# shenwei356/bio

Measured on AMD Instinct MI355X. Metric: Gbases/s hashed (k=21 ntHash + minimizer), higher is better.
Workload: dtype u64

## Files before the change

bio_amd/csrc/kernels_pk.hpp:

```cpp
#pragma once
#include <utility>

#include "kernels_fast.hpp"

namespace bsk {

template <int... Is, class F>
__device__ __forceinline__ void pk_unroll_impl(std::integer_sequence<int, Is...>, F &&f) {
    (f(std::integral_constant<int, Is>{}), ...);
}
template <int N, class F>
__device__ __forceinline__ void pk_unroll(F &&f) {
    pk_unroll_impl(std::make_integer_sequence<int, N>{}, f);
}

#ifndef BSK_PK_ROWS
#define BSK_PK_ROWS 58
#endif
struct PkLds {
    static constexpr int PR = BSK_PK_ROWS;
    static constexpr int ROW = 33;
    static constexpr int TAB = 0;
    static constexpr int TAB2 = 320;
    static constexpr int NHEADS = (32 * (PR - 1)) / 64 + 2;
    static constexpr int HEADS = 0;
    static constexpr int CTAB = 256;
    static constexpr int SH = 768;
    static constexpr int SP = SH + (PR + 1) * ROW * 8;
    static constexpr int TOTAL = (SP + (PR + 1) * ROW * 2 + 15) & ~15;
    static_assert(NHEADS * 8 <= CTAB && CTAB + 512 <= SH && TAB2 + 256 <= SH && TOTAL <= 20480, "PkLds");
};

struct PkTabs {
    u32x4 row;
    u32 at;
    __device__ __forceinline__ void init(int k, int lane, u32 tab = (u32)PkLds::TAB, u32 tab2 = (u32)PkLds::TAB2) {
        row = (u32x4){0, 0, 0, 0};
        at = 0xffffffffu;
        if (lane < 20) {
            const unsigned out = (unsigned)lane >> 2, in = (unsigned)lane & 3u;
            u64 f = seed_fwd_code(in);
            u64 r = rol64(seed_rev_code(in), (unsigned)(k - 1));
            if (out < 4) {
                f ^= rol64(seed_fwd_code(out), (unsigned)k);
                r ^= ror64(seed_rev_code(out), 1);
            }
            row = (u32x4){(u32)f, (u32)(f >> 32), (u32)r, (u32)(r >> 32)};
            at = tab + (u32)lane * 16u;
        } else if (lane >= 32 && lane < 48) {
            const unsigned c0 = (unsigned)lane & 3u, c1 = ((unsigned)lane >> 2) & 3u;
            const u64 f = rol64(seed_fwd_code(c0), 1) ^ seed_fwd_code(c1);
            const u64 r = ror64(rol64(seed_rev_code(c0), (unsigned)(k - 1)), 1) ^ rol64(seed_rev_code(c1), (unsigned)(k - 1));
            row = (u32x4){(u32)f, (u32)(f >> 32), (u32)r, (u32)(r >> 32)};
            at = tab2 + (u32)(lane - 32) * 16u;
        }
    }
    __device__ __forceinline__ void write(LDSQ char *ldsq) const {
        if (at != 0xffffffffu) *reinterpret_cast<LDSQ u32x4 *>(ldsq + at) = row;
        wave_sync_lds();
    }
};

template <int W>
struct PkCfg {
    static constexpr int XC = W > 12 ? 4 : W;
};

#define PKNW 16
typedef u32 u32x16 __attribute__((ext_vector_type(16)));
struct PkWords {
    u32x4 a, b, c, d;
};
__device__ __forceinline__ PkWords pk_load_words(const u32 *p) {
    PkWords r;
    asm volatile("global_load_dwordx4 %0, %4, off\n\tglobal_load_dwordx4 %1, %4, off offset:16\n\t"
                 "global_load_dwordx4 %2, %4, off offset:32\n\tglobal_load_dwordx4 %3, %4, off offset:48"
                 : "=&v"(r.a), "=&v"(r.b), "=&v"(r.c), "=&v"(r.d)
                 : "v"(p));
    return r;
}
__device__ __forceinline__ u64 pk_load_u64(const u64 *p) {
    u64 r;
    asm volatile("global_load_dwordx2 %0, %1, off" : "=&v"(r) : "v"(p));
    return r;
}
__device__ __forceinline__ void pk_wait_loads(u64 &d0, u64 &d1) { asm volatile("s_waitcnt vmcnt(0)" : "+v"(d0), "+v"(d1)::"memory"); }
__device__ __forceinline__ void pk_wait_loads(PkWords &p) { asm volatile("s_waitcnt vmcnt(0)" : "+v"(p.a), "+v"(p.b), "+v"(p.c), "+v"(p.d)::"memory"); }
__device__ __forceinline__ void pk_ticket_async(u32 *ticket, u32 &t) {
    u64 ex;
    asm volatile("s_mov_b64 %1, exec\n\ts_mov_b64 exec, 1\n\tglobal_atomic_add %0, %2, %3, off sc0\n\ts_mov_b64 exec, %1"
                 : "+v"(t), "=&s"(ex)
                 : "v"(ticket), "v"(1u)
                 : "memory");
}
__device__ __forceinline__ void pk_wait_loads(PkWords &p, u64 &d0, u32 &f, u32 &t) {
    asm volatile("s_waitcnt vmcnt(0)" : "+v"(p.a), "+v"(p.b), "+v"(p.c), "+v"(p.d), "+v"(d0), "+v"(f), "+v"(t)::"memory");
}
__device__ __forceinline__ u32 pk_load_u8(const u8 *p) {
    u32 r;
    asm volatile("global_load_ubyte %0, %1, off" : "=&v"(r) : "v"(p));
    return r;
}
template <int W, bool LONG, class LY_ = PkLds, bool RINGM = false, bool SELM = false>
struct PkMin {
    typedef LY_ LY;
    const u32 *__restrict__ w;
    LDSQ char *lds;
    int k, lane;
    u32 nk;
    u32 fl, fh_, rl, rh_;
    u32 S[W];
    u64 H[W];
    u32 SB[W];
    u32 P, bm, tmin;
    u32 nsel;
    u32 slot, spare;
    u32 glo, gspan;
    u32 c8000;
    int sstep;
    u32 send;
    u32 in_lo, in_hi, out_lo, out_hi;
    u32x4 pw;
    u32x16 wr;
    static constexpr bool POS2 = !RINGM && !SELM;
    u32 i2;

    __device__ __forceinline__ void set_words(const PkWords &p) {
        wr = (u32x16){p.a.x, p.a.y, p.a.z, p.a.w, p.b.x, p.b.y, p.b.z, p.b.w, p.c.x, p.c.y, p.c.z, p.c.w, p.d.x, p.d.y, p.d.z, p.d.w};
    }
    __device__ __forceinline__ void word2(u32 i, u32 &lo, u32 &hi) const {
        const u32 iu = (u32)__builtin_amdgcn_readfirstlane((int)i);
        if (!LONG || iu + 1 < (u32)PKNW) {
            lo = wr[iu], hi = wr[iu + 1];
        } else {
            lo = w[iu], hi = w[iu + 1];
        }
    }
    __device__ __forceinline__ u32 word(u32 i) const {
        const u32 iu = (u32)__builtin_amdgcn_readfirstlane((int)i);
        if constexpr (RINGM) {
            if (iu < 4u) return iu == 0 ? pw.x : iu == 1 ? pw.y : iu == 2 ? pw.z : pw.w;
            return w[iu];
        }
        if (!LONG || iu < (u32)PKNW) return wr[iu];
        return w[iu];
    }
    __device__ __forceinline__ void load_block_words(u32 i0) {
        const u32 t0 = i0 + (u32)k - 1, p0 = i0 - 1;
        in_lo = w[t0 >> 4];
        in_hi = w[(t0 >> 4) + 1];
        out_lo = w[p0 >> 4];
        out_hi = w[(p0 >> 4) + 1];
    }
    __device__ __forceinline__ void load_block0_words() {
        const u32 t0 = (u32)k - 1;
        in_lo = word(t0 >> 4);
        in_hi = word((t0 >> 4) + 1);
        out_lo = word(0);
        out_hi = word(1);
    }
    __device__ __forceinline__ void roll(u32x4 x) {
        const u32 a = __builtin_amdgcn_alignbit(fl, fh_, 31), b = __builtin_amdgcn_alignbit(fh_, fl, 31);
        const u32 c = __builtin_amdgcn_alignbit(rh_, rl, 1), d = __builtin_amdgcn_alignbit(rl, rh_, 1);
        fl = a ^ x.x;
        fh_ = b ^ x.y;
        rl = c ^ x.z;
        rh_ = d ^ x.w;
    }
    __device__ __forceinline__ void roll2(u32x4 x) {
        const u32 a = __builtin_amdgcn_alignbit(fl, fh_, 30), b = __builtin_amdgcn_alignbit(fh_, fl, 30);
        const u32 c = __builtin_amdgcn_alignbit(rh_, rl, 2), d = __builtin_amdgcn_alignbit(rl, rh_, 2);
        fl = a ^ x.x;
        fh_ = b ^ x.y;
        rl = c ^ x.z;
        rh_ = d ^ x.w;
    }

    __device__ __forceinline__ void guard() {
        if constexpr (RINGM || SELM) return;
        const bool in = slot - glo <= gspan;
        slot = in ? slot : spare;
        sstep = in ? sstep : 0;
    }
    template <int IDX, int O>
    __device__ __forceinline__ void emit(u32 pbase) {
        if constexpr (!SELM) emit_staged<IDX, O>(pbase);
    }
    template <int IDX, int O>
    __device__ __forceinline__ void emit_staged(u32 pbase) {
        const u32 b = (bm >> IDX) & 1u;
        u32 pv;
        if constexpr (POS2) {
            (void)pbase;
            pv = SB[O];
        } else {
            asm("v_add3_u32 %0, %1, %2, %3" : "=v"(pv) : "v"(SB[O]), "s"(pbase), "n"(O));
        }
#if defined(PK_MASKST)
        {
            const u32 a0 = (u32)(uintptr_t)(lds + LY::SH) + slot, a1 = (u32)(uintptr_t)(lds + LY::SP) + (slot >> 2);
            u64 sv;
            asm volatile("v_cmp_ne_u32_e32 vcc, 0, %1\n\ts_and_saveexec_b64 %0, vcc\n\tds_write_b64 %2, %3\n\tds_write_b16 %4, %5\n\ts_mov_b64 exec, %0"
                         : "=&s"(sv) : "v"(b), "v"(a0), "v"(H[O]), "v"(a1), "v"(pv) : "vcc", "memory");
        }
#elif defined(PK_NOPOS)
        *reinterpret_cast<LDSQ u64 *>(lds + LY::SH + slot) = H[O];
#ifdef PK_STRMASK
        asm volatile("" ::"v"(pv));
#endif
#elif !defined(PK_NOSTAGE)
        *reinterpret_cast<LDSQ u64 *>(lds + LY::SH + slot) = H[O];
        *reinterpret_cast<LDSQ u16 *>(lds + LY::SP + (slot >> 2)) = (u16)pv;
#else
        asm volatile("" ::"v"(H[O]), "v"(pv), "v"(slot));
#endif
        asm("v_mad_i32_i24 %0, %1, %2, %0" : "+v"(slot) : "v"(b), "v"(sstep));
        if constexpr (RINGM) slot = slot == send ? (u32)lane * 8u : slot;
    }

    template <bool FIRST, bool RAG, int PAR>
    __device__ __forceinline__ void block(u32 i0, u32 okbit, bool suffix) {
        constexpr int CB = PAR * 16, PB = (1 - PAR) * 16;
        constexpr int XC = PkCfg<W>::XC;
        const u32 t0 = i0 + (u32)k - 1, p0 = FIRST ? 0u : i0 - 1u;
        u32 in_lo, in_hi, out_lo, out_hi;
        if constexpr (RINGM) {
            in_lo = this->in_lo, in_hi = this->in_hi, out_lo = this->out_lo, out_hi = this->out_hi;
            load_block_words(i0 + (u32)W);
        } else {
            word2(t0 >> 4, in_lo, in_hi);
            word2(p0 >> 4, out_lo, out_hi);
        }
        const u32 cinb = __builtin_amdgcn_alignbit(in_hi, in_lo, (t0 & 15) * 2);
        u32 coutb;
        if (FIRST) coutb = out_lo << 2;
        else coutb = __builtin_amdgcn_alignbit(out_hi, out_lo, (p0 & 15) * 2);
        const u32 E = (cinb & 0x33333333u) | ((coutb & 0x33333333u) << 2);
        const u32 O = ((cinb >> 2) & 0x33333333u) | (coutb & 0xCCCCCCCCu);
        const u32 E4 = E << 4, O4 = O << 4;
        u32x4 xs[W];
        auto fetch = [&](int o0) {
#pragma unroll
            for (int o = o0; o < o0 + XC && o < W; ++o) {
                const int j = o >> 1;
                const u32 src = (j & 1) ? ((o & 1) ? O : E) : ((o & 1) ? O4 : E4);
                u32 a;
                switch (j >> 1) {
                    case 0: asm("v_and_b32_sdwa %0, %1, %2 dst_sel:DWORD dst_unused:UNUSED_PAD src0_sel:BYTE_0 src1_sel:DWORD" : "=v"(a) : "v"(src), "s"(0xF0u)); break;
                    case 1: asm("v_and_b32_sdwa %0, %1, %2 dst_sel:DWORD dst_unused:UNUSED_PAD src0_sel:BYTE_1 src1_sel:DWORD" : "=v"(a) : "v"(src), "s"(0xF0u)); break;
                    case 2: asm("v_and_b32_sdwa %0, %1, %2 dst_sel:DWORD dst_unused:UNUSED_PAD src0_sel:BYTE_2 src1_sel:DWORD" : "=v"(a) : "v"(src), "s"(0xF0u)); break;
                    default: asm("v_and_b32_sdwa %0, %1, %2 dst_sel:DWORD dst_unused:UNUSED_PAD src0_sel:BYTE_3 src1_sel:DWORD" : "=v"(a) : "v"(src), "s"(0xF0u)); break;
                }
                if (FIRST && o == 0) a = 0x100u | (a & 0x30u);
#ifndef PK_NOTAB
                xs[o] = *reinterpret_cast<LDSQ const u32x4 *>(lds + LY::TAB + a);
#else
                xs[o] = (u32x4){a, a ^ E, a + O, a ^ cinb};
#endif
            }
        };
        fetch(0);
        if (XC < W) fetch(XC);
        const u32 pbase = (u32)__builtin_amdgcn_readfirstlane((int)(i0 - (u32)W));
        if constexpr (POS2) {
            i2 = 2u * i0;
            asm volatile("" : "+v"(i2));
        }
        if (!FIRST) guard();
        u32 vb = 0;
        if (RAG && !FIRST) {
            const int left = (int)nk - (int)i0;
            const u32 nv = (u32)(left < 0 ? 0 : left > W ? W : left);
            vb = (1u << nv) - 1u;
        }
        pk_unroll<W>([&](auto oc) {
            constexpr int o = decltype(oc)::value;
            if (XC < W && o && o % XC == 0 && o + XC < W) {
                __builtin_amdgcn_sched_barrier(0);
                fetch(o + XC);
            }
            roll(xs[o]);
            if (!FIRST) this->template emit<PB + o, o>(pbase);
            const lmask rev = lt64(rl, rh_, fl, fh_);
            const u32 hl = sel(rev, rl, fl), hh = sel(rev, rh_, fh_);
            if constexpr (POS2) {
                lmask co;
                asm("v_addc_co_u32_e64 %0, %1, %2, %3, %4" : "=v"(SB[o]), "=s"(co) : "n"(2 * o), "v"(i2), "s"(rev));
            } else {
                asm("v_cndmask_b32_e64 %0, 0, %1, %2" : "=v"(SB[o]) : "v"(c8000), "s"(rev));
            }
            H[o] = ((u64)hh << 32) | hl;
            u32 pk;
            asm("v_and_or_b32 %0, %1, %2, %3" : "=v"(pk) : "v"(hh), "s"(0xffffffe0u), "n"(CB + o));
            if (o == 0) {
                P = pk;
            } else {
#ifndef PK_NOTIE
                const u32 d = pk ^ P;
                tmin = tmin < d ? tmin : d;
#endif
                P = P < pk ? P : pk;
            }
            if (!FIRST || o == W - 1) {
                u32 m = P;
                if constexpr (o != W - 1) {
#ifndef PK_NOTIE
                    const u32 d = P ^ S[o + 1];
                    tmin = tmin < d ? tmin : d;
#endif
                    m = P < S[o + 1] ? P : S[o + 1];
                }
                u32 one = 1u;
                if (FIRST) one = okbit;
                else if (RAG) one = (vb >> o) & 1u;
                bm |= one << (m & 31u);
            }
            S[o] = pk;
        });
        if (suffix) {
#pragma unroll
            for (int q = W - 2; q >= 0; --q) {
#ifndef PK_NOTIE
                const u32 d = S[q] ^ S[q + 1];
                tmin = tmin < d ? tmin : d;
#endif
                S[q] = S[q] < S[q + 1] ? S[q] : S[q + 1];
            }
        }
        if constexpr (SELM) {
            if (!FIRST) {
                const u32 wsel = (bm >> PB) & ((1u << W) - 1u);
                *reinterpret_cast<LDSQ u32 *>(lds + LY::MASK + (i0 / (u32)W - 1u) * 256u + (u32)lane * 4u) = wsel;
                nsel += (u32)__builtin_popcount(wsel);
            }
        }
        if (!FIRST) bm &= PAR ? 0xffff0000u : 0x0000ffffu;
    }

    template <int PAR>
    __device__ __forceinline__ void drain(u32 i0) {
        if constexpr (SELM) {
            const u32 wsel = (bm >> (PAR * 16)) & ((1u << W) - 1u);
            *reinterpret_cast<LDSQ u32 *>(lds + LY::MASK + (i0 / (u32)W) * 256u + (u32)lane * 4u) = wsel;
            nsel += (u32)__builtin_popcount(wsel);
            return;
        }
        const u32 pbase = (u32)__builtin_amdgcn_readfirstlane((int)i0);
        guard();
        pk_unroll<W>([&](auto oc) {
            constexpr int o = decltype(oc)::value;
            this->template emit<PAR * 16 + o, o>(pbase);
        });
    }

    __device__ __forceinline__ void begin(u32 slot0, int step, u32 col8) {
        fl = fh_ = rl = rh_ = 0;
        bm = 0;
        nsel = 0;
        c8000 = 0x8000u;
        asm volatile("" : "+v"(c8000));
        tmin = 0xffffffffu;
        slot = slot0;
        sstep = step;
        if constexpr (RINGM) {
            (void)col8;
            spare = glo = gspan = 0;
            send = (u32)(LY::ROWS * LY::ROW * 8) + (u32)lane * 8u;
        } else {
            spare = (u32)(LY::PR * LY::ROW * 8) + col8;
            send = 0;
            constexpr u32 RB = (u32)(LY::ROW * 8);
            glo = step < 0 ? col8 + (u32)(W - 1) * RB : col8;
            gspan = (u32)(LY::PR - W) * RB + (step < 0 ? 0u : RB);
        }
        if constexpr (RINGM) load_block0_words();
        for (int t0 = 0; t0 < k - 1; t0 += 16) {
            const u32 word = this->word((u32)t0 >> 4);
            const int nb = (k - 1 - t0) < 16 ? (k - 1 - t0) : 16;
            int j = 0;
            for (; j + 8 <= nb; j += 8) {
                const u32 sub = word >> (2 * j);
                const u32x4 x0 = *reinterpret_cast<LDSQ const u32x4 *>(lds + LY::TAB2 + ((sub & 0xf) << 4));
                const u32x4 x1 = *reinterpret_cast<LDSQ const u32x4 *>(lds + LY::TAB2 + (sub & 0xf0));
                const u32x4 x2 = *reinterpret_cast<LDSQ const u32x4 *>(lds + LY::TAB2 + ((sub & 0xf00) >> 4));
                const u32x4 x3 = *reinterpret_cast<LDSQ const u32x4 *>(lds + LY::TAB2 + ((sub & 0xf000) >> 8));
                roll2(x0);
                roll2(x1);
                roll2(x2);
                roll2(x3);
            }
            for (; j + 2 <= nb; j += 2) roll2(*reinterpret_cast<LDSQ const u32x4 *>(lds + LY::TAB2 + (((word >> (2 * j)) & 0xf) << 4)));
            for (; j < nb; ++j) roll(*reinterpret_cast<LDSQ const u32x4 *>(lds + LY::TAB + 256 + (((word >> (2 * j)) & 3) << 4)));
        }
    }

    __device__ __forceinline__ void run(u32 nk_max, bool ok, u32 nk_min, u32 slot0, int step, u32 col8) {
        begin(slot0, step, col8);
        block<true, false, 0>(0, ok ? 1u : 0u, nk_max > (u32)W);
        u32 i0 = W;
        int last_par = 0;
        for (;;) {
            if (i0 >= nk_max) break;
            {
                const bool more = i0 + W < nk_max;
                if (i0 + W <= nk_min) block<false, false, 1>(i0, 1u, more);
                else block<false, true, 1>(i0, 1u, more);
            }
            i0 += W;
            last_par = 1;
            if (i0 >= nk_max) break;
            {
                const bool more = i0 + W < nk_max;
                if (i0 + W <= nk_min) block<false, false, 0>(i0, 1u, more);
                else block<false, true, 0>(i0, 1u, more);
            }
            i0 += W;
            last_par = 0;
        }
        if (last_par) drain<1>(i0 - W);
        else drain<0>(i0 - W);
    }
};

template <int U, class LY = PkLds, bool POS2 = false>
__device__ __forceinline__ void pk_copyout(char *lds, int lane, u32 cnt, u32 excl, u32 T, u64 base, const KArgs &a) {
    constexpr int NH = LY::NHEADS;
    u64 *s_heads = reinterpret_cast<u64 *>(lds + LY::HEADS);
    u64 *s_tab64 = reinterpret_cast<u64 *>(lds + LY::CTAB);
    const u64 nzmask = __builtin_amdgcn_ballot_w64(cnt > 0);
    if (lane < NH) s_heads[lane] = 0;
    wave_sync_lds();
    if (cnt > 0) {
        constexpr int RB = LY::ROW * 8;
        const int col8 = (lane & 31) * 8;
        const int S = lane < 32 ? RB : -RB;
        const int A = lane < 32 ? col8 - (int)excl * RB : col8 + ((int)(LY::PR - 1) + (int)excl) * RB;
        const u32 rk = __builtin_amdgcn_mbcnt_hi((u32)(nzmask >> 32), __builtin_amdgcn_mbcnt_lo((u32)nzmask, 0));
        s_tab64[rk] = ((u64)(u32)S << 32) | (u32)A;
        if (excl) atomicOr(&s_heads[(excl - 1u) >> 6], 1ULL << ((excl - 1u) & 63u));
    }
    wave_sync_lds();
    const u64 hw = lane < NH ? s_heads[lane] : 0ULL;
    const u32 hw_lo = (u32)hw, hw_hi = (u32)(hw >> 32);
    u32 heads_before = 0;
    const char *sh = lds + LY::SH, *sp = lds + LY::SP;
    u64 *const gh = a.hash + base;
    u32 *const gp = a.pos + base;
    auto trip = [&](u32 t0, auto check) {
        constexpr bool CHECK = decltype(check)::value;
        u32 rank[U];
#pragma unroll
        for (int j = 0; j < U; ++j) {
            const u32 c = (t0 >> 6) + j;
            const u32 mlo = (u32)__builtin_amdgcn_readlane((int)hw_lo, (int)c), mhi = (u32)__builtin_amdgcn_readlane((int)hw_hi, (int)c);
            rank[j] = (__builtin_amdgcn_mbcnt_hi(mhi, __builtin_amdgcn_mbcnt_lo(mlo, 0u)) << 3) + (heads_before << 3);
            heads_before += (u32)__builtin_popcountll(((u64)mhi << 32) | mlo);
        }
        u64 ent[U];
#pragma unroll
        for (int j = 0; j < U; ++j) ent[j] = *reinterpret_cast<const u64 *>(reinterpret_cast<const char *>(s_tab64) + rank[j]);
        if constexpr (U == 8) {
            __builtin_amdgcn_sched_barrier(0);
            asm volatile("" ::"v"(ent[0]), "v"(ent[1]), "v"(ent[2]), "v"(ent[3]), "v"(ent[4]), "v"(ent[5]), "v"(ent[6]), "v"(ent[7]));
            __builtin_amdgcn_sched_barrier(0);
        }
        u64 hv[U];
        u32 pv[U];
#pragma unroll
        for (int j = 0; j < U; ++j) {
            const u32 t = t0 + 64 * j + lane;
            const int off = __mul24((int)t, (int)(u32)(ent[j] >> 32)) + (int)(u32)ent[j];
            const u32 so = (!CHECK || t < T) ? (u32)off : 0u;
            hv[j] = *reinterpret_cast<const u64 *>(sh + so);
            if constexpr (POS2) pv[j] = *reinterpret_cast<const u16 *>(sp + (so >> 2));
            else pv[j] = (u32)(int)*reinterpret_cast<const short *>(sp + (so >> 2));
        }
        if constexpr (U == 8) {
            __builtin_amdgcn_sched_barrier(0);
            asm volatile("" ::"v"(hv[0]), "v"(hv[1]), "v"(hv[2]), "v"(hv[3]), "v"(hv[4]), "v"(hv[5]), "v"(hv[6]), "v"(hv[7]), "v"(pv[0]), "v"(pv[1]),
                         "v"(pv[2]), "v"(pv[3]), "v"(pv[4]), "v"(pv[5]), "v"(pv[6]), "v"(pv[7]));
            __builtin_amdgcn_sched_barrier(0);
        }
#pragma unroll
        for (int j = 0; j < U; ++j) {
            const u32 t = t0 + 64 * j + lane;
#ifdef PK_NOSTORE
            asm volatile("" ::"v"(hv[j]), "v"(pv[j]));
#else
            if (!CHECK || t < T) {
#ifndef PK_NOHASHST
                __builtin_nontemporal_store(hv[j], &gh[t]);
#else
                asm volatile("" ::"v"(hv[j]));
#endif
#ifndef PK_NOPOSST
                __builtin_nontemporal_store(POS2 ? __builtin_amdgcn_alignbit(pv[j], pv[j], 1) : pv[j] & 0x80007fffu, &gp[t]);
#else
                asm volatile("" ::"v"(pv[j]));
#endif
            }
#endif
        }
    };
    u32 t0 = 0;
    for (; t0 + 64 * U <= T; t0 += 64 * U) trip(t0, std::false_type{});
    if (t0 < T) trip(t0, std::true_type{});
    wave_sync_lds();
}

#ifndef PK_TICKET
#define PK_TICKET 8u
#endif
template <int W, bool LONG>
__global__ __launch_bounds__(64, 2) void k_minimizer_pk(KArgs a) {
    typedef PkLds LY;
    __shared__ __attribute__((aligned(16))) char lds[LY::TOTAL];
    LDSQ char *const ldsq = (LDSQ char *)lds;
    const int lane = lane_id();
    PkTabs tabs;
    tabs.init(a.k, lane);
#ifdef PK_STAGGER
    for (u32 i = (((blockIdx.x * 2654435761u) >> 24) * (u32)PK_STAGGER) >> 8; i; --i) __builtin_amdgcn_s_sleep(32);
#endif
    const u64 slab = (u64)64 * BSK_FAST_CAP;
    const u32 col8 = (u32)(lane & 31) * 8u;
    constexpr u32 RB = (u32)(LY::ROW * 8);
    const u32 top = (u32)(LY::PR - 1) * RB + col8;
    u64 d_n1 = 0, d_cur = 0;
    PkWords pw_cur = {{0, 0, 0, 0}, {0, 0, 0, 0}, {0, 0, 0, 0}, {0, 0, 0, 0}};
    bool have = false;
    const u32 lseg = a.fixcap / a.list_grid;
    u32 lcur = 0;
    const u32 tku = a.tk ? a.tk : PK_TICKET;
    const bool ahead = tku >= 3u;
    u32 tv = 0;
    u32 nt = ~0u;
    for (u32 unit = next_ticket(a.ticket, lane) * tku, uend = unit + tku; unit < a.nunits; ++unit, ({
             if (unit == uend) {
                 unit = ahead ? nt : next_ticket(a.ticket, lane) * tku;
                 uend = unit + tku;
             }
         })) {
        const u64 r = (u64)unit * 64 + lane;
        const u64 u2 = (!ahead || unit + 2u < uend) ? (u64)unit + 2u : (u64)nt + (unit + 2u - uend);
        const bool nxt = unit + 1 != uend ? unit + 1 < a.nunits : ahead && nt < a.nunits;
        const bool ask = ahead && unit + 3u == uend;
        const u64 rmax = a.n - 1;
        if (!have) {
            d_cur = pk_load_u64(a.desc + (r < rmax ? r : rmax));
            d_n1 = pk_load_u64(a.desc + (r + 64 < rmax ? r + 64 : rmax));
            pk_wait_loads(d_cur, d_n1);
            pw_cur = pk_load_words(a.words + (d_cur >> 24));
            pk_wait_loads(pw_cur);
        }
        PkWords pw_n1 = pk_load_words(a.words + (d_n1 >> 24));
        const u64 r2 = u2 * 64 + lane;
        u64 d_n2 = pk_load_u64(a.desc + (r2 < rmax ? r2 : rmax));
        u32 rfl = pk_load_u8(a.rflags ? a.rflags + (r < rmax ? r : rmax) : reinterpret_cast<const u8 *>(a.desc));
        if (ask) pk_ticket_async(a.ticket, tv);
        const u64 d = d_cur;
        const PkWords pw = pw_cur;
        const u64 off = d >> 24, L = desc_len(a, d);
        const u64 ro = out_index(a, r, d);
        const bool ok = r < a.n && L >= (u64)a.circ_ext && (L - (u64)a.circ_ext) + 1 >= (u64)a.k + (u64)W;
        const u32 nk = ok ? (u32)(L - a.k + 1) : 0u;
        const u32 nk_max = wave_max_u32(nk);
        const u32 nk_min = ~wave_max_u32(~(ok ? nk : 0xffffffffu));
        u32 cnt = 0, tmin_lane = 0xffffffffu;
        if (nk_max) {
            tabs.write(ldsq);
            PkMin<W, LONG> pm;
            pm.w = a.words + off;
            pm.set_words(pw);
            pm.lds = ldsq;
            pm.k = a.k;
            pm.lane = lane;
            pm.nk = nk;
            const u32 spare = (u32)LY::PR * RB + col8;
            pm.run(nk_max, ok, nk_min, !ok ? spare : lane < 32 ? col8 : top, !ok ? 0 : lane < 32 ? (int)RB : -(int)RB, col8);
            if (ok) cnt = (lane < 32 ? pm.slot - col8 : top - pm.slot) / RB;
            tmin_lane = pm.tmin;
        }
        pk_wait_loads(pw_n1, d_n2, rfl, tv);
        if (ask) nt = (u32)__builtin_amdgcn_readfirstlane((int)tv) * tku;
        d_cur = d_n1;
        pw_cur = pw_n1;
        d_n1 = d_n2;
        have = nxt;
        const u32 cnt_pair = cnt + (u32)__builtin_amdgcn_ds_bpermute((lane ^ 32) * 4, (int)cnt);
        u64 bad = __builtin_amdgcn_ballot_w64(cnt_pair >= (u32)LY::PR);
        u64 tied = __builtin_amdgcn_ballot_w64(ok && tmin_lane < 32u);
#if defined(PK_NOSTAGE) || defined(PK_NOTIE) || defined(PK_NOTAB) || defined(PK_NOCOPY) || defined(PK_NOSTORE) || defined(PK_NOFB)
        bad = 0;
        tied = 0;
#endif
        const u64 redo = bad | tied;
        if (redo) {
            list_append(a, a.rlist, lseg, lcur, redo, lane, r);
            if ((redo >> lane) & 1) cnt = 0;
        }
        const u32 incl = wave_incl_scan_u32(cnt, lane);
        const u32 excl = incl - cnt;
        const u32 T = wave_bcast_u32(incl, 63);
        const u64 base = (u64)unit * slab;
#ifndef PK_NOCOPY
#ifndef PK_CU
#define PK_CU 8
#endif
        if (T) pk_copyout<PK_CU, LY, PkMin<W, LONG>::POS2>(lds, lane, cnt, excl, T, base, a);
#endif
        if (r < a.n) {
            if (!((redo >> lane) & 1)) a.refs[ro] = ((base + excl) << 24) | cnt;
            u8 sbyte = ok ? BSK_ST_OK : BSK_ST_SHORT;
            if (ok && a.rflags) sbyte |= (u8)rfl;
            a.status[ro] = sbyte;
        }
    }
    list_close(a.rlist, lseg, lcur, lane);
}

#ifdef BSK_IMPL_PK
#ifndef BSK_PK_WS
#define BSK_PK_WS(X) X(2) X(3) X(4) X(5) X(6) X(7) X(8) X(9) X(10) X(11) X(12) X(13)
#endif
bool pk_minimizer_supported(int w) { return w >= 2 && w <= 13; }
u32 pk_minimizer_short_bases() { return 16u * (PKNW - 1); }
int pk_minimizer_blocks_per_cu(int w) {
    int nb = 0;
    hipError_t e = hipErrorInvalidValue;
    switch (w) {
#define X(WW) \
    case WW: e = hipOccupancyMaxActiveBlocksPerMultiprocessor(&nb, k_minimizer_pk<WW, false>, 64, 0); break;
        BSK_PK_WS(X)
#undef X
        default: break;
    }
    if (e != hipSuccess || nb < 1) {
        (void)hipGetLastError();
        nb = 1;
    }
    return nb;
}
void pk_minimizer_list_launch(int w, int grid, hipStream_t stream, const KArgs &a) {
    switch (w) {
#define X(WW) \
    case WW: hipLaunchKernelGGL((k_minimizer_dense<WW, true>), dim3(grid), dim3(64), 0, stream, a); break;
        BSK_PK_WS(X)
#undef X
        default: break;
    }
}
void pk_minimizer_launch(int w, bool long_reads, int grid, hipStream_t stream, const KArgs &a) {
    switch (w) {
#define X(WW)                                                                                               \
    case WW:                                                                                                \
        if (long_reads) {                                                                                   \
            hipLaunchKernelGGL((k_minimizer_pk<WW, true>), dim3(grid), dim3(64), 0, stream, a);             \
        } else {                                                                                            \
            hipLaunchKernelGGL((k_minimizer_pk<WW, false>), dim3(grid), dim3(64), 0, stream, a);            \
        }                                                                                                   \
        hipLaunchKernelGGL((k_minimizer_dense<WW, true>), dim3(grid), dim3(64), 0, stream, a);              \
        break;
        BSK_PK_WS(X)
#undef X
        default: break;
    }
}
#endif

}
```

Measured before the change: 1234.

## Split block loop into steady-state and ragged phases with carried bit offsets

Splits block() into steps/suffix_pass/tail and restructures run() into a steady-state loop over full, non-ragged block pairs, followed by a ragged tail loop. Bit offsets into the packed sequence (t2, p2) are carried in scalar registers instead of being recomputed from i0 each block. The POS2 position counter is advanced incrementally. The suffix pass skips index 0, which appears unused. This targets per-block branching and scalar address arithmetic, at the cost of more code and a riskier loop-boundary calculation.

```diff
diff --git a/bio_amd/csrc/kernels_pk.hpp b/bio_amd/csrc/kernels_pk.hpp
--- a/bio_amd/csrc/kernels_pk.hpp
+++ b/bio_amd/csrc/kernels_pk.hpp
@@ -220,21 +220,30 @@
 
     template <bool FIRST, bool RAG, int PAR>
     __device__ __forceinline__ void block(u32 i0, u32 okbit, bool suffix) {
+        static_assert(!POS2, "POS2 (k_minimizer_pk): i2 is advanced by run()");
+        const u32 t0 = i0 + (u32)k - 1, p0 = FIRST ? 0u : i0 - 1u;
+        steps<FIRST, RAG, PAR>(2u * t0, 2u * p0, i0, okbit);
+        if (suffix) suffix_pass();
+        tail<FIRST, PAR>(i0);
+    }
+
+    template <bool FIRST, bool RAG, int PAR>
+    __device__ __forceinline__ void steps(u32 t2, u32 p2, u32 i0, u32 okbit) {
         constexpr int CB = PAR * 16, PB = (1 - PAR) * 16;
         constexpr int XC = PkCfg<W>::XC;
-        const u32 t0 = i0 + (u32)k - 1, p0 = FIRST ? 0u : i0 - 1u;
+        constexpr int O2 = PAR ? 0 : 2 * W;
         u32 in_lo, in_hi, out_lo, out_hi;
         if constexpr (RINGM) {
             in_lo = this->in_lo, in_hi = this->in_hi, out_lo = this->out_lo, out_hi = this->out_hi;
             load_block_words(i0 + (u32)W);
         } else {
-            word2(t0 >> 4, in_lo, in_hi);
-            word2(p0 >> 4, out_lo, out_hi);
-        }
-        const u32 cinb = __builtin_amdgcn_alignbit(in_hi, in_lo, (t0 & 15) * 2);
+            word2(t2 >> 5, in_lo, in_hi);
+            word2(p2 >> 5, out_lo, out_hi);
+        }
+        const u32 cinb = __builtin_amdgcn_alignbit(in_hi, in_lo, t2 & 31u);
         u32 coutb;
         if (FIRST) coutb = out_lo << 2;
-        else coutb = __builtin_amdgcn_alignbit(out_hi, out_lo, (p0 & 15) * 2);
+        else coutb = __builtin_amdgcn_alignbit(out_hi, out_lo, p2 & 31u);
         const u32 E = (cinb & 0x33333333u) | ((coutb & 0x33333333u) << 2);
         const u32 O = ((cinb >> 2) & 0x33333333u) | (coutb & 0xCCCCCCCCu);
         const u32 E4 = E << 4, O4 = O << 4;
@@ -261,11 +270,8 @@
         };
         fetch(0);
         if (XC < W) fetch(XC);
-        const u32 pbase = (u32)__builtin_amdgcn_readfirstlane((int)(i0 - (u32)W));
-        if constexpr (POS2) {
-            i2 = 2u * i0;
-            asm volatile("" : "+v"(i2));
-        }
+        u32 pbase = 0;
+        if constexpr (!POS2) pbase = (u32)__builtin_amdgcn_readfirstlane((int)(i0 - (u32)W));
         if (!FIRST) guard();
         u32 vb = 0;
         if (RAG && !FIRST) {
@@ -285,7 +291,7 @@
             const u32 hl = sel(rev, rl, fl), hh = sel(rev, rh_, fh_);
             if constexpr (POS2) {
                 lmask co;
-                asm("v_addc_co_u32_e64 %0, %1, %2, %3, %4" : "=v"(SB[o]), "=s"(co) : "n"(2 * o), "v"(i2), "s"(rev));
+                asm("v_addc_co_u32_e64 %0, %1, %2, %3, %4" : "=v"(SB[o]), "=s"(co) : "n"(O2 + 2 * o), "v"(i2), "s"(rev));
             } else {
                 asm("v_cndmask_b32_e64 %0, 0, %1, %2" : "=v"(SB[o]) : "v"(c8000), "s"(rev));
             }
@@ -317,16 +323,22 @@
             }
             S[o] = pk;
         });
-        if (suffix) {
+    }
+
+    __device__ __forceinline__ void suffix_pass() {
 #pragma unroll
-            for (int q = W - 2; q >= 0; --q) {
+        for (int q = W - 2; q >= 1; --q) {
 #ifndef PK_NOTIE
-                const u32 d = S[q] ^ S[q + 1];
-                tmin = tmin < d ? tmin : d;
-#endif
-                S[q] = S[q] < S[q + 1] ? S[q] : S[q + 1];
-            }
-        }
+            const u32 d = S[q] ^ S[q + 1];
+            tmin = tmin < d ? tmin : d;
+#endif
+            S[q] = S[q] < S[q + 1] ? S[q] : S[q + 1];
+        }
+    }
+
+    template <bool FIRST, int PAR>
+    __device__ __forceinline__ void tail(u32 i0) {
+        constexpr int PB = (1 - PAR) * 16;
         if constexpr (SELM) {
             if (!FIRST) {
                 const u32 wsel = (bm >> PB) & ((1u << W) - 1u);
@@ -334,7 +346,7 @@
                 nsel += (u32)__builtin_popcount(wsel);
             }
         }
-        if (!FIRST) bm &= PAR ? 0xffff0000u : 0x0000ffffu;
+        if (!FIRST) asm("v_and_b32_e32 %0, %1, %0" : "+v"(bm) : "n"(PAR ? 0xffff0000u : 0x0000ffffu));
     }
 
     template <int PAR>
@@ -394,28 +406,57 @@
         }
     }
 
+    static constexpr bool CARRY = !SELM;
+    __device__ __forceinline__ void advance(u32 &i0, u32 &t2, u32 &p2) const {
+        if constexpr (CARRY) {
+            t2 += 2u * W, p2 += 2u * W;
+            asm volatile("" : "+s"(t2), "+s"(p2));
+            i0 = (p2 >> 1) + 1u;
+        } else {
+            i0 += W;
+            t2 = 2u * (i0 + (u32)k - 1u), p2 = 2u * (i0 - 1u);
+        }
+    }
+
     __device__ __forceinline__ void run(u32 nk_max, bool ok, u32 nk_min, u32 slot0, int step, u32 col8) {
         begin(slot0, step, col8);
-        block<true, false, 0>(0, ok ? 1u : 0u, nk_max > (u32)W);
+        if constexpr (POS2) i2 = (u32)(-2 * W);
+        steps<true, false, 0>(2u * ((u32)k - 1u), 0u, 0u, ok ? 1u : 0u);
+        if (nk_max <= (u32)W) {
+            drain<0>(0);
+            return;
+        }
+        suffix_pass();
         u32 i0 = W;
-        int last_par = 0;
+        u32 t2 = 2u * ((u32)W + (u32)k - 1u), p2 = 2u * ((u32)W - 1u);
+        if constexpr (CARRY) asm volatile("" : "+s"(t2), "+s"(p2));
+        const int lim = 2 * ((int)__builtin_amdgcn_readfirstlane((int)(nk_min < 0x8000u ? nk_min : 0x8000u)) - 2 * W - 1);
+        while ((int)p2 < lim) {
+            if constexpr (POS2) asm("v_add_u32_e32 %0, %1, %0" : "+v"(i2) : "n"(4 * W));
+            steps<false, false, 1>(t2, p2, i0, 1u);
+            suffix_pass();
+            tail<false, 1>(i0);
+            advance(i0, t2, p2);
+            steps<false, false, 0>(t2, p2, i0, 1u);
+            suffix_pass();
+            tail<false, 0>(i0);
+            advance(i0, t2, p2);
+        }
+        int last_par;
         for (;;) {
-            if (i0 >= nk_max) break;
-            {
-                const bool more = i0 + W < nk_max;
-                if (i0 + W <= nk_min) block<false, false, 1>(i0, 1u, more);
-                else block<false, true, 1>(i0, 1u, more);
-            }
-            i0 += W;
+            if constexpr (POS2) asm("v_add_u32_e32 %0, %1, %0" : "+v"(i2) : "n"(4 * W));
+            steps<false, true, 1>(t2, p2, i0, 1u);
+            tail<false, 1>(i0);
+            advance(i0, t2, p2);
             last_par = 1;
             if (i0 >= nk_max) break;
-            {
-                const bool more = i0 + W < nk_max;
-                if (i0 + W <= nk_min) block<false, false, 0>(i0, 1u, more);
-                else block<false, true, 0>(i0, 1u, more);
-            }
-            i0 += W;
+            suffix_pass();
+            steps<false, true, 0>(t2, p2, i0, 1u);
+            tail<false, 0>(i0);
+            advance(i0, t2, p2);
             last_par = 0;
+            if (i0 >= nk_max) break;
+            suffix_pass();
         }
         if (last_par) drain<1>(i0 - W);
         else drain<0>(i0 - W);
```

Measured after the change: 1252, median of 6. 1.5% higher.
